# DataZooDE/anofox-forecast

Hardware: AMD Instinct MI355X
Metric: series/sec fit+forecast, AutoETS h=28 on M5-shape batches (higher is better)
Workload: dtype f64

## Files before the change

### anofox-forecast_amd/csrc/host_api.hip

```cpp
#include <hip/hip_runtime.h>

#include <algorithm>
#include <cctype>
#include <atomic>
#include <memory>
#include <unordered_map>
#include <chrono>
#include <cmath>
#include <condition_variable>
#include <mutex>
#include <cstdio>
#include <cstdlib>
#include <cstring>
#include <limits>
#include <map>
#include <stdexcept>
#include <string>
#include <system_error>
#include <thread>
#include <vector>

#include "classic_device.hpp"
#include "host_semantics.hpp"
#include "kernels.hpp"
// ... 59 lines not shown
    unsigned short *d_yc16 = nullptr;
    size_t yc_cells = 0;
    unsigned int *d_misfit = nullptr;
    unsigned int h_misfit[2] = {1u, 1u};
    int y_type = 0;
    unsigned long long *d_wave_trace = nullptr;
    unsigned long long *d_lane_stats = nullptr;
    double *d_yhat = nullptr, *d_lo = nullptr, *d_hi = nullptr;
    int32_t *d_model_code = nullptr, *d_status = nullptr, *d_detail = nullptr, *d_passes_total = nullptr, *d_evals_total = nullptr;
    uint32_t *d_mask = nullptr;
    int32_t *d_len_group = nullptr;
    int32_t *d_count = nullptr;
    int32_t *d_pos_map = nullptr, *d_pos_cnt = nullptr, *d_notpos = nullptr;
    double *d_ypos = nullptr;
    bool use_pos = false;
    bool none_pos = false;
    std::vector<anofox::FitArgs> insp_args;
    std::vector<anofox::FitLaunchers> insp_fns;
    std::vector<int> insp_spec, insp_stream;
    bool insp_ok = false;
    int insp_m = 1;
    int32_t live_pos = -1, live_all = -1;
    int arima_method = 0;
    size_t ar_ws_bytes = 0;
    double *ar_w = nullptr, *ar_wmean = nullptr, *ar_wsd = nullptr, *ar_l0 = nullptr, *ar_l1 = nullptr, *ar_x = nullptr, *ar_aicc = nullptr;
    int32_t *ar_wlen = nullptr, *ar_d = nullptr, *ar_D = nullptr, *ar_order = nullptr, *ar_status = nullptr, *ar_evals = nullptr, *ar_passes = nullptr, *ar_models = nullptr;
    StreamSet *sset = nullptr;
    hipStream_t own_stream = nullptr;
    hipStream_t aux[N_AUX_STREAMS] = {};
    hipEvent_t ev_start = nullptr, ev_stop = nullptr, ev_fit0 = nullptr, ev_fit1 = nullptr, ev_fork = nullptr;
    hipEvent_t ev_join[N_AUX_STREAMS] = {};
    struct Lane {
        double *ybuf = nullptr;
        size_t ybuf_cols = 0;
        int32_t *map[2] = {nullptr, nullptr};
        int32_t *cnt = nullptr;
        anofox::NmStateBuf st{};
        double *nm_scratch = nullptr;
        size_t nm_scratch_doubles = 0;
    } lanes[N_AUX_STREAMS];
    anofox::FitArgs *d_group_tab = nullptr, *h_group_tab = nullptr;
    size_t group_tab_cap = 0;
    hipEvent_t ev_group_tab = nullptr;
    hipStream_t last_stream = nullptr;
    bool ran = false, timed_fit = false;
    uint32_t fit_launches = 0;
    uint64_t n_problems = 0;
    Tunables tun;
    int seq_rounds = 3;
    int seq_rounds_env = -1;
    int spec_below_md = 8192;
    anofox::NmStateBuf classic_st{};
    int32_t *d_classic_status = nullptr, *classic_map[2] = {nullptr, nullptr}, *classic_cnt = nullptr;
    double *d_classic_ybuf = nullptr;
    size_t classic_ybuf_cols = 0;
    std::vector<void *> retired;
    int merged_m_max = 0;
    int32_t *d_m_col = nullptr;
    int spec2_below_md = 2048;
    int spec2_below = 1024;
    int spec_below = 8192;
    bool use_gather = false;
    double gather_budget = 0.0;
    bool sd_in_final = false;
    double *d_ring = nullptr;
    size_t ring_elems = 0;
    double *d_prep_scratch = nullptr;
    size_t prep_scratch_elems = 0;
    bool fixed_params = false;
    double fixed_x[4] = {0.0, 0.0, 0.0, 0.0};
    int32_t *d_im_level = nullptr, *d_im_gmax = nullptr;
    double *d_im_fc = nullptr;
    size_t im_fc_elems = 0;
// ... 124 lines not shown
{
    if (!b->sset) return;
    stream_set_give(b->sset);
    b->sset = nullptr; b->own_stream = nullptr; b->last_stream = nullptr; b->ran = false;
    for (auto &q : b->aux) q = nullptr;
}

void free_batch_buffers(AnofoxHipBatch *b)
{
    auto F = [](void *p) { dev_free(p, true); };
    if (b->owns_y) F(b->d_y);
    pin_free(b->h_stage);
    if (b->owns_len) F(b->d_len);
    F(b->d_mean); F(b->d_sd); F(b->d_fig_add); F(b->d_fig_mul); F(b->d_l0); F(b->d_b0); F(b->d_flags);
    F(b->d_aicc); F(b->d_yhat_slots); F(b->d_status_slots); F(b->d_evals_slots); F(b->d_iters_slots);
    F(b->d_passes_slots); F(b->d_slot_spec); F(b->d_lane_stats); F(b->d_wave_trace); F(b->d_yc32); F(b->d_yc16); F(b->d_misfit);
    F(b->d_yhat); F(b->d_lo); F(b->d_hi); F(b->d_model_code); F(b->d_status); F(b->d_detail);
    F(b->classic_st.sim); F(b->classic_st.fs); F(b->classic_st.phase); F(b->classic_st.evals); F(b->classic_st.iters); F(b->classic_st.passes); F(b->classic_st.done);
    F(b->d_classic_ybuf); F(b->d_classic_status); F(b->classic_map[0]); F(b->classic_map[1]); F(b->classic_cnt);
    for (void *p : b->retired) F(p);
    b->retired.clear();
    F(b->d_m_col); F(b->d_ring); F(b->d_prep_scratch);
    F(b->d_group_tab); pin_free(b->h_group_tab); b->d_group_tab = b->h_group_tab = nullptr; b->group_tab_cap = 0;
    if (b->ev_group_tab) { (void)hipEventDestroy(b->ev_group_tab); b->ev_group_tab = nullptr; }
    F(b->d_im_level); F(b->d_im_gmax); F(b->d_im_fc);
    F(b->d_th_sidx); F(b->d_th_adj);
    if (b->owns_exog) { F((void *)b->d_exog_x); F((void *)b->d_exog_f); }
    b->d_exog_x = b->d_exog_f = nullptr; b->owns_exog = false; b->exog_k = 0;
    F(b->d_exog_b0); F(b->d_exog_beta); F(b->d_exog_used);
    F(b->d_passes_total); F(b->d_evals_total); F(b->d_mask); F(b->d_len_group); F(b->d_count); F(b->d_pos_map); F(b->d_pos_cnt); F(b->d_notpos); F(b->d_ypos);
    F(b->ar_w); F(b->ar_wmean); F(b->ar_wsd); F(b->ar_l0); F(b->ar_l1); F(b->ar_x); F(b->ar_aicc); F(b->ar_wlen); F(b->ar_d); F(b->ar_D);
    F(b->ar_order); F(b->ar_status); F(b->ar_evals); F(b->ar_passes); F(b->ar_models);
    batch_detach_streams(b);
    for (auto &l : b->lanes) {
        F(l.ybuf); l.ybuf_cols = 0; F(l.map[0]); F(l.map[1]); F(l.cnt);
        F(l.st.sim); F(l.st.fs); F(l.st.phase); F(l.st.evals); F(l.st.iters); F(l.st.passes); F(l.st.done);
        F(l.nm_scratch); l.nm_scratch_doubles = 0;
    }
}

int max_slots_for(const Plan &p)
{
    if (p.model == M_AutoETS) return 30;
    if (p.model == M_ETS && p.ets_spec_id >= 0) return 1;
    return 0;
}

void alloc_common(AnofoxHipBatch *b)
{
    const size_t n = b->n, ld = b->ld, h = (size_t)std::max(b->h, 0);
    b->d_mean = dalloc<double>(ld);
    b->d_sd = dalloc<double>(ld);
    b->d_flags = dalloc<uint32_t>(ld);
    b->d_yhat = dalloc<double>(n * h);
    b->d_lo = dalloc<double>(n * h);
    b->d_hi = dalloc<double>(n * h);
    b->d_model_code = dalloc<int32_t>(ld);
    b->d_status = dalloc<int32_t>(ld);
    b->d_detail = dalloc<int32_t>(ld);
    b->d_passes_total = dalloc<int32_t>(ld);
    b->d_evals_total = dalloc<int32_t>(ld);
    b->d_mask = dalloc<uint32_t>(ld);
    b->d_len_group = dalloc<int32_t>(ld);
    b->d_count = dalloc<int32_t>(2);
    if (b->plan.model == M_AutoETS) {
        b->d_pos_map = dalloc<int32_t>(ld); b->d_pos_cnt = dalloc<int32_t>(2); b->d_notpos = dalloc<int32_t>(ld);
    }
    if (is_intermittent_model(b->plan.model)) {
// ... 2 lines not shown
    }
    if (is_theta_model(b->plan.model)) b->d_th_adj = dalloc<int32_t>(ld);
    if (b->plan.model == M_AutoARIMA) {
        const size_t T = std::max<size_t>(b->t_max, 1);
        b->ar_ws_bytes = arima_workspace_bytes((int)b->n, (int)T);
        b->ar_w = (double *)dalloc<char>(b->ar_ws_bytes);
        HIPCHECK(hipMemset(b->ar_w, 0, b->ar_ws_bytes));
        b->ar_wmean = dalloc<double>(ld); b->ar_wsd = dalloc<double>(ld); b->ar_l0 = dalloc<double>(ld); b->ar_l1 = dalloc<double>(ld);
        b->ar_x = dalloc<double>(6 * ld); b->ar_aicc = dalloc<double>(ld);
        b->ar_wlen = dalloc<int32_t>(ld); b->ar_d = dalloc<int32_t>(ld); b->ar_D = dalloc<int32_t>(ld); b->ar_order = dalloc<int32_t>(5 * ld);
        b->ar_status = dalloc<int32_t>(ld); b->ar_evals = dalloc<int32_t>(ld); b->ar_passes = dalloc<int32_t>(ld); b->ar_models = dalloc<int32_t>(ld);
        HIPCHECK(hipMemset(b->ar_wlen, 0, ld * sizeof(int32_t)));
    }
    HIPCHECK(hipMemset(b->d_model_code, 0, ld * sizeof(int32_t)));
    HIPCHECK(hipMemset(b->d_detail, 0, ld * sizeof(int32_t)));
    HIPCHECK(hipMemset(b->d_passes_total, 0, ld * sizeof(int32_t)));
    HIPCHECK(hipMemset(b->d_evals_total, 0, ld * sizeof(int32_t)));
    HIPCHECK(hipMemset(b->d_mask, 0, ld * sizeof(uint32_t)));
    b->n_slots_cap = max_slots_for(b->plan);
    if (b->n_slots_cap > 0) {
        const size_t S = (size_t)b->n_slots_cap;
        b->d_l0 = dalloc<double>(9 * ld);
        b->d_b0 = dalloc<double>(9 * ld);
        b->d_aicc = dalloc<double>(S * ld);
        b->d_yhat_slots = dalloc<double>(S * n * h);
        b->d_status_slots = dalloc<int32_t>(S * ld);
        b->d_evals_slots = dalloc<int32_t>(S * ld);
        b->d_iters_slots = dalloc<int32_t>(S * ld);
        b->d_passes_slots = dalloc<int32_t>(S * ld);
        b->d_slot_spec = dalloc<int32_t>(S);
        b->d_lane_stats = dalloc<unsigned long long>(2 * S);
        HIPCHECK(hipMemset(b->d_lane_stats, 0, 2 * S * sizeof(unsigned long long)));
        const int n_lanes = std::min<int>(N_AUX_STREAMS, b->n_slots_cap);
        for (int q = 0; q < n_lanes; q++) {
            auto &l = b->lanes[q];
            l.map[0] = dalloc<int32_t>(ld);
            l.map[1] = dalloc<int32_t>(ld);
            l.cnt = dalloc<int32_t>(3);
            l.st.sim = dalloc<double>(20 * ld);
            l.st.fs = dalloc<double>(5 * ld);
            l.st.phase = dalloc<int32_t>(ld);
            l.st.evals = dalloc<int32_t>(ld);
            l.st.iters = dalloc<int32_t>(ld);
            l.st.passes = dalloc<int32_t>(ld);
            l.st.done = dalloc<int32_t>(ld);
        }
    }
    batch_attach_streams(b);
}

void ensure_fig(AnofoxHipBatch *b, int m)
{
    if (m <= b->fig_m) return;
    if (b->d_fig_add) b->retired.push_back(b->d_fig_add);
    if (b->d_fig_mul) b->retired.push_back(b->d_fig_mul);
    b->d_fig_add = nullptr; b->d_fig_mul = nullptr; b->fig_m = 0;
    b->d_fig_add = dalloc<double>((size_t)m * b->ld);
    b->d_fig_mul = dalloc<double>((size_t)m * b->ld);
    b->fig_m = m;
}

double *ensure_ring(AnofoxHipBatch *b, size_t elems)
{
    if (b->ring_elems < elems) {
        if (b->d_ring) b->retired.push_back(b->d_ring);
        b->d_ring = nullptr; b->ring_elems = 0;
        b->d_ring = dalloc<double>(elems);
        b->ring_elems = elems;
    }
    return b->d_ring;
}
// ... 126 lines not shown
}

void batch_detect_periods(AnofoxHipBatch *b)
{
    std::vector<int32_t> per(b->n, 0);
    batch_attach_streams(b);
    detect_periods_block(b->d_y, b->ld, b->d_len, b->n, std::max<size_t>(b->t_max, 1), per.data(), b->own_stream);
    b->h_period.assign(b->n, 1);
    for (size_t s = 0; s < b->n; s++) b->h_period[s] = per[s] > 0 ? per[s] : 1;
}

void run_classic(AnofoxHipBatch *b, int kind, const int32_t *d_len, int m, int optimized, double alpha, int min_len,
                 const uint32_t *mask, uint32_t want, int32_t code, bool write_code, hipStream_t st)
{
    ClassicArgs a{};
    a.y = b->d_y; a.ld = b->ld; a.len = d_len; a.n_series = (int)b->n;
    a.m = m; a.h = b->h; a.optimized = optimized; a.fixed_alpha = alpha;
    a.mask = mask; a.want = want; a.min_len = min_len;
    a.yhat = b->d_yhat; a.status = b->d_detail; a.passes = b->d_passes_total;
    a.model_code = code; a.model_code_out = write_code ? b->d_model_code : nullptr;
    a.ring_scratch = nullptr;
    a.m_col = (kind == CK_HW || kind == CK_SEASONAL_ES) ? b->d_m_col : nullptr;
    const bool optimise = kind == CK_HOLT || kind == CK_HW || optimized != 0;
    if (optimise) {
        const size_t n = b->n, ld = b->ld;
        if (!b->classic_st.sim) {
            b->classic_st.sim = dalloc<double>(12 * ld); b->classic_st.fs = dalloc<double>(4 * ld);
            b->classic_st.phase = dalloc<int32_t>(ld); b->classic_st.evals = dalloc<int32_t>(ld); b->classic_st.iters = dalloc<int32_t>(ld);
            b->classic_st.passes = dalloc<int32_t>(ld); b->classic_st.done = dalloc<int32_t>(ld);
            b->d_classic_status = dalloc<int32_t>(ld);
            b->classic_map[0] = dalloc<int32_t>(ld); b->classic_map[1] = dalloc<int32_t>(ld); b->classic_cnt = dalloc<int32_t>(3);
        }
        double *ybuf = (b->n_slots_cap > 0 && b->use_gather) ? b->lanes[0].ybuf : nullptr;
        size_t ybuf_cols = ybuf ? b->lanes[0].ybuf_cols : ld;
        if (!ybuf) {
            const double per_col = (double)std::max<size_t>(b->t_max, 1) * 8.0;
            const size_t cols = (size_t)std::min((double)ld, 32.0 * 1073741824.0 / per_col) / 64 * 64;
            if (cols >= 1024 || cols >= ld) {
                if (!b->d_classic_ybuf) { b->d_classic_ybuf = dalloc<double>(std::max<size_t>(b->t_max, 1) * cols); b->classic_ybuf_cols = cols; }
                ybuf = b->d_classic_ybuf;
                ybuf_cols = b->classic_ybuf_cols;
            }
        }
        const bool seasonal = kind == CK_HW || kind == CK_SEASONAL_ES;
        FitArgs f{};
        f.y = b->d_y; f.ld = ld; f.len = d_len; f.n_series = (int)n; f.t_rows = (int)std::max<size_t>(b->t_max, 1);
        f.m = seasonal ? std::max(m, 1) : 1; f.h = b->h;
        f.flags = b->d_flags; f.fig = nullptr; f.fig_ld = ld;
        f.status = b->d_classic_status; f.st = b->classic_st;
        f.mask = mask; f.want = want; f.min_len = min_len;
        f.m_col = a.m_col;
        const bool merged = f.m_col != nullptr;
        FitLaunchers fns = classic_fit_launcher(kind, (merged && f.m == 7) ? 8 : f.m);
        if (!fns.round_seq || !fns.round_spec || !fns.round_spec2 || !fns.round_auto) throw HipFail{"no round kernel for this model"};
        if (f.m > ETS_LDS_PERIOD) {
            const size_t wg = merged ? n : std::max<size_t>((n + 15) / 16, std::min<size_t>(n, 1024));
            f.ring_scratch = ensure_ring(b, wg * (size_t)f.m * 64u);
            f.ring_scratch_doubles = wg * (size_t)f.m * 64u;
        }
        static const int BUDGET[] = {24, 24, 24, 24, 48, 48, 96, 192, 1024};
        const bool tiny = n <= TINY_BATCH_PROBLEMS;
        const int n_rounds = tiny ? 1 : (merged ? (n > 4096 ? 4 : 3) : (int)(sizeof BUDGET / sizeof BUDGET[0]));
        for (int r = 0; r < n_rounds; r++) {
            f.first_round = (r == 0);
            f.spec_below = -1; f.spec2_below = -1;
            f.gathered = 0;
            f.y_round = b->d_y; f.ld_round = ld; f.series_of = nullptr; f.n_active = nullptr;
// ... 291 lines not shown
                all_additive = false;
        int64_t additive_live = 0;
        for (size_t oi = 0; oi < order.size(); oi++)
            if (!dead[oi] && !spec_has_mult(specs[order[oi]])) additive_live += b->live_all >= 0 ? (int64_t)b->live_all : (int64_t)n;
        int64_t all_live = 0;
        for (size_t oi = 0; oi < order.size(); oi++)
            if (!dead[oi]) all_live += (spec_has_mult(specs[order[oi]]) && b->live_pos >= 0) ? (int64_t)b->live_pos : (b->live_all >= 0 ? (int64_t)b->live_all : (int64_t)n);
        const bool on = b->tun.k4 > 0 || (b->tun.k4 < 0 && yt == YT_F64 && ((all_additive && additive_live >= 131072) || all_live >= 524288));
        for (size_t oi = 0; oi < order.size(); oi++)
            k4[oi] = on && !dead[oi] && !b->fixed_params && !spec_has_mult(specs[order[oi]]) && fns[oi].round_k4 && fns[oi].round_auto_k4;
    }
    std::vector<char> fill_spec4(order.size(), 0);
    bool fill_mode = false;
    {
        int64_t lanes = 0;
        std::vector<int64_t> live_of(order.size(), 0);
        for (size_t oi = 0; oi < order.size(); oi++) {
            if (dead[oi]) continue;
            live_of[oi] = (spec_has_mult(specs[order[oi]]) && b->live_pos >= 0) ? (int64_t)b->live_pos : (b->live_all >= 0 ? (int64_t)b->live_all : (int64_t)n);
            lanes += live_of[oi];
        }
        const int64_t resident = 2 * 1024 * 64;
        const bool tiny_batch = (uint64_t)n * order.size() <= (uint64_t)TINY_BATCH_PROBLEMS;
        fill_mode = b->tun.fill_policy > 0 && !tiny_batch && !b->fixed_params && order.size() > 1 && b->seq_rounds_env < 0 && b->seq_rounds == 0 &&
                    lanes * 4 > 8 * resident;
        if (fill_mode) {
            const int64_t target = resident * (int64_t)b->tun.fill_target / 100;
            for (size_t oi = 0; oi < order.size(); oi++) {
                if (dead[oi] || k4[oi]) continue;
                if (lanes + 3 * live_of[oi] <= target) { fill_spec4[oi] = 1; lanes += 3 * live_of[oi]; }
            }
        }
    }
    if (b->use_gather && !b->fixed_params) {
        const size_t T = std::max<size_t>(b->t_max, 1);
        std::vector<size_t> need(order.size(), 0);
        double total = 0.0;
        for (size_t oi = 0; oi < order.size(); oi++) {
            if (dead[oi]) continue;
            size_t c = (b->use_pos && args[oi].need_positive && b->live_pos >= 0) ? (size_t)b->live_pos : n;
            need[oi] = std::min(ld, (c + 63) / 64 * 64);
            total += (double)need[oi] * (double)T * 8.0;
        }
        const double scale = total > b->gather_budget ? b->gather_budget / total : 1.0;
        for (size_t oi = 0; oi < order.size(); oi++) {
            if (dead[oi]) continue;
            auto &lane = b->lanes[oi % (size_t)n_lanes];
            size_t cols = scale < 1.0 ? (size_t)((double)need[oi] * scale) / 64 * 64 : need[oi];
            if (b->tun.gather_cols > 0) cols = std::min<size_t>(need[oi], (size_t)b->tun.gather_cols / 64 * 64);
            if (cols < need[oi] && cols < 1024 && b->tun.gather_cols <= 0) cols = 0;
            if (lane.ybuf && lane.ybuf_cols >= cols) continue;
            if (lane.ybuf) {
                HIPCHECK(hipDeviceSynchronize());
                dev_free(lane.ybuf, true);
                lane.ybuf = nullptr; lane.ybuf_cols = 0;
            }
            while (cols >= 64) {
                try { lane.ybuf = dalloc<double>(T * cols); lane.ybuf_cols = cols; break; }
                catch (const HipFail &f) {
                    if (!f.oom) throw;
                    cols = cols / 2 / 64 * 64;
                    if (cols < 1024) cols = 0;
                }
            }
        }
    }
    const bool tiny = (uint64_t)n * order.size() <= (uint64_t)TINY_BATCH_PROBLEMS;
    const int total_rounds = b->fixed_params ? 0 : (tiny ? 1 : n_rounds);
    enum { RK_SEQ, RK_SPEC, RK_SPEC2, RK_AUTO, RK_K4, RK_AUTO_K4 };
    std::vector<int> group_of(order.size(), -1);
    std::vector<std::vector<size_t>> groups;
    std::vector<int> group_stream;
    std::vector<GroupLaunchFn> group_fn;
    std::vector<size_t> slot_of(order.size(), 0);
    size_t n_slots = 0;
    bool grouped = b->tun.group_launch > 0 && !inline_stream && !tiny && !merged && !b->fixed_params && total_rounds > 0;
    if (grouped) {
        GroupLaunchFn fn[N_GROUP_CLASSES];
        for (int c = 0; c < N_GROUP_CLASSES; c++) fn[c] = ets_group_launcher(c, m, yt);
        std::vector<size_t> of_class[N_GROUP_CLASSES];
        for (size_t oi = 0; oi < order.size() && grouped; oi++) {
            if (dead[oi]) continue;
            const int c = ets_group_class(specs[order[oi]]);
            if (c < 0 || !fn[c] || fns[oi].nm_scratch_per_wg != 0) grouped = false;
            else of_class[c].push_back(oi);
        }
        if (grouped) {
            auto add = [&](const std::vector<size_t> &sl, int c) {
                if (sl.empty()) return;
                if (sl.size() > (size_t)GROUP_MAX_SLOTS) throw HipFail{"launch_fit_slots: more specs in one group than GROUP_MAX_SLOTS"};
                groups.push_back(sl); group_fn.push_back(fn[c]);
// ... 60 lines not shown
            const bool spec_mode = r >= b->seq_rounds;
            a.first_round = (r == 0);
            a.wave_trace_tag = ((unsigned long long)specs[order[oi]] << 32) | ((unsigned long long)r << 16);
            a.wave_prio = (int)oi < b->tun.prio_top ? std::max(1, 3 - (int)oi) : 0;
            a.spec_below = -1; a.spec2_below = -1;
            a.gathered = 0;
            if (tiny) {
                a.y_round = b->d_y; a.ld_round = ld; a.series_of = nullptr; a.n_active = nullptr;
                a.budget = 1 << 30; a.budget_seq = a.budget;
                run_round(oi, RK_SPEC2, a, sq, r);
                b->fit_launches++;
                return;
            }
            if (r == 0 && b->use_pos && a.need_positive) {
                if (emit)
                    hipLaunchKernelGGL(retire_nonpositive_kernel, dim3((unsigned)((n + 255) / 256)), dim3(256), 0, sq, (int)n, d_len, b->d_notpos,
                                       a.status, lane.st.done, lane.st.passes, lane.st.evals, lane.st.iters);
                a.series_of = b->d_pos_map; a.n_active = b->d_pos_cnt;
                if (b->d_ypos) { a.y_round = b->d_ypos; a.ld_round = ld; a.gathered = 1; a.gather_cap = (int)ld; }
                else { a.y_round = b->d_y; a.ld_round = ld; }
            } else if (r == 0) {
                a.y_round = a.y; a.ld_round = ld; a.series_of = nullptr; a.n_active = nullptr;
            } else {
                const int32_t *prev_map = (r == 1) ? nullptr : lane.map[(r - 1) & 1];
                const int32_t *prev_cnt = (r == 1) ? nullptr : lane.cnt + ((r - 1) % 3);
                if (emit && !grouped && r == 1) HIPCHECK(hipMemsetAsync(lane.cnt, 0, 3 * sizeof(int32_t), sq));
                if (emit && !grouped) launch_compact(prev_map, prev_cnt, (int)n, lane.st.done, lane.map[r & 1], lane.cnt + (r % 3), sq, lane.cnt + ((r + 1) % 3));
                if (emit && grouped) {
                    const int k = gc.n_slots++;
                    gc.prev[k] = prev_map; gc.n_prev[k] = prev_cnt; gc.done[k] = lane.st.done;
                    gc.next[k] = lane.map[r & 1]; gc.n_next[k] = lane.cnt + (r % 3); gc.n_clear[k] = lane.cnt + ((r + 1) % 3);
                }
                a.series_of = lane.map[r & 1]; a.n_active = lane.cnt + (r % 3);
                if (b->use_gather && lane.ybuf) {
                    if (emit && !grouped)
                        launch_gather_columns(a.y, ld, lane.map[r & 1], lane.cnt + (r % 3), (int)n, (int)b->t_max, lane.ybuf, lane.ybuf_cols, sq,
                                              (int)lane.ybuf_cols, ybytes);
                    if (emit && grouped) {
                        const int k = gg.n_slots++;
                        gg.series_of[k] = lane.map[r & 1]; gg.n_active[k] = lane.cnt + (r % 3);
                        gg.out[k] = lane.ybuf; gg.ld_out[k] = lane.ybuf_cols; gg.cap[k] = (int)lane.ybuf_cols;
                        gg_cols = std::max(gg_cols, (int)std::min<size_t>(n, lane.ybuf_cols));
                    }
                    a.y_round = lane.ybuf; a.ld_round = lane.ybuf_cols; a.gathered = 1; a.gather_cap = (int)lane.ybuf_cols;
                } else {
                    a.y_round = a.y; a.ld_round = ld;
                }
            }
            const int s2 = (spec_trend_idx(specs[order[oi]]) == 4) ? b->spec2_below_md : b->spec2_below;
            if (fill_mode && !k4[oi]) {
                const int64_t live_i = (spec_has_mult(specs[order[oi]]) && b->live_pos >= 0) ? (int64_t)b->live_pos : (b->live_all >= 0 ? (int64_t)b->live_all : (int64_t)n);
                const int s2v = (int)std::max<int64_t>(32, std::min<int64_t>(s2 > 0 ? s2 : 32, live_i / std::max(1, b->tun.fill_s2_div)));
                a.budget = BUDGET[r]; a.budget_seq = (BUDGET[r] * 7) / 4;
                if (r == 0) {
                    if (fill_spec4[oi]) run_round(oi, RK_SPEC, a, sq, r);
                    else { a.budget = a.budget_seq; run_round(oi, RK_SEQ, a, sq, r); }
                } else {
                    a.spec_below = fill_spec4[oi] ? 0x7fffffff : (int)std::max<int64_t>(64, live_i / std::max(1, b->tun.fill_late_div));
                    a.spec2_below = s2v;
                    run_round(oi, RK_AUTO, a, sq, r);
                }
                if (!grouped) b->fit_launches++;
                return;
            }
            if (k4[oi]) {
                a.budget = BUDGET[r]; a.budget_seq = BUDGET[r];
                const int64_t live = b->live_all >= 0 ? b->live_all : (int64_t)n;
                const int sb = ((int)oi < b->tun.k4_top && b->tun.k4_top_below > 0) ? b->tun.k4_top_below : b->spec_below;
                if (r == 0) run_round(oi, live > sb ? RK_K4 : RK_SPEC, a, sq, r);
                else {
                    a.spec_below = sb; a.spec2_below = s2 > 0 ? s2 : -1;
                    run_round(oi, RK_AUTO_K4, a, sq, r);
                }
            } else if (r == 0 || b->seq_rounds_env >= 0 || b->seq_rounds == 0) {
                a.budget = spec_mode ? BUDGET[r] : (BUDGET[r] * 7) / 4;
                if (spec_mode && r > 0 && s2 > 0) {
                    a.spec_below = 0x7fffffff; a.spec2_below = s2; a.budget_seq = a.budget;
                    run_round(oi, RK_AUTO, a, sq, r);
                } else
                    run_round(oi, spec_mode ? RK_SPEC : RK_SEQ, a, sq, r);
            } else {
                a.spec_below = (spec_trend_idx(specs[order[oi]]) == 4) ? b->spec_below_md : b->spec_below;
                a.spec2_below = s2 > 0 ? s2 : -1;
                if ((int)oi < b->tun.top_boost_n) {
                    a.spec_below = (int)std::min<int64_t>(0x7fffffff, (int64_t)a.spec_below * b->tun.top_boost_pct / 100);
                    if (a.spec2_below > 0) a.spec2_below = (int)std::min<int64_t>(0x7fffffff, (int64_t)a.spec2_below * b->tun.top_boost_pct / 100);
                }
                a.budget_seq = (BUDGET[r] * 7) / 4;
                a.budget = BUDGET[r];
                run_round(oi, RK_AUTO, a, sq, r);
            }
            if (!grouped) b->fit_launches++;
    };
    if (grouped) {
        const size_t cells = (size_t)total_rounds * n_slots;
        if (b->ev_group_tab) HIPCHECK(hipEventSynchronize(b->ev_group_tab));
        else HIPCHECK(hipEventCreateWithFlags(&b->ev_group_tab, hipEventDisableTiming));
        if (b->group_tab_cap < cells) {
            if (b->d_group_tab) b->retired.push_back(b->d_group_tab);
            pin_free(b->h_group_tab);
            b->d_group_tab = nullptr; b->h_group_tab = nullptr; b->group_tab_cap = 0;
            b->d_group_tab = dalloc<FitArgs>(cells);
            b->h_group_tab = (FitArgs *)pin_alloc_bytes(cells * sizeof(FitArgs));
            b->group_tab_cap = cells;
        }
        slot_blocks.assign(cells, 0); slot_k4.assign(cells, 0);
        emit = false;
        for (int r = 0; r < total_rounds; r++) for (size_t oi = 0; oi < order.size(); oi++) enqueue_round(r, oi);
        emit = true;
        HIPCHECK(hipMemcpyAsync(b->d_group_tab, b->h_group_tab, cells * sizeof(FitArgs), hipMemcpyHostToDevice, st));
        HIPCHECK(hipEventRecord(b->ev_group_tab, st));
        HIPCHECK(hipEventRecord(b->ev_fork, st));
        for (int q : group_stream) HIPCHECK(hipStreamWaitEvent(b->aux[q], b->ev_fork, 0));
    } else
        for (int i = 0; i < n_fork; i++) HIPCHECK(hipStreamWaitEvent(b->aux[i], b->ev_fit0, 0));
    for (size_t oi = 0; oi < order.size(); oi++)
        if (dead[oi]) {
            const FitArgs &a = args[oi];
            hipLaunchKernelGGL(retire_nonpositive_kernel, dim3((unsigned)((n + 255) / 256)), dim3(256), 0, spec_stream(stream_of[oi]), (int)n, d_len,
                               b->d_notpos, a.status, a.st.done, a.st.passes, a.st.evals, a.st.iters, a.aicc, a.passes, a.evals, a.iters);
        }
    if (b->fixed_params) {
        for (size_t oi = 0; oi < order.size(); oi++) {
            const int id = specs[order[oi]];
            FitArgs &a = args[oi];
            double x[4] = {0.0, 0.0, 0.0, 0.0};
            int d = 0;
            x[d++] = b->fixed_x[0];
            if (spec_trend_idx(id) != 0) x[d++] = b->fixed_x[1];
            if (spec_season(id) != 0) x[d++] = b->fixed_x[2];
            if (spec_trend_idx(id) == 2 || spec_trend_idx(id) == 4) x[d++] = b->fixed_x[3];
            hipLaunchKernelGGL(ets_fixed_setup_kernel, dim3((unsigned)((n + 255) / 256)), dim3(256), 0, spec_stream(stream_of[oi]), (int)n, ld, d_len,
                               b->d_flags, spec_season(id) != 0 ? 1 : 0, a.m, a.n_param, a.need_positive, d, x[0], x[1], x[2], x[3], a.status,
                               a.st.sim, a.st.evals, a.st.iters, a.st.passes, a.st.done);
        }
        LAUNCHCHECK("ETS fixed-parameter setup");
    }
    auto enqueue_group_round = [&](const int r, const size_t g) {
        hipStream_t sg = b->aux[group_stream[g]];
        if (r == 0) {
            int32_t *zero[GROUP_MAX_SLOTS] = {};
            for (size_t k = 0; k < groups[g].size(); k++) zero[k] = b->lanes[groups[g][k] % (size_t)n_lanes].cnt;
            launch_group_zero3((int)groups[g].size(), zero, sg);
        }
        gc = GroupCompactArgs{}; gc.n_series = (int)n;
        gg = GroupGatherArgs{}; gg.t_max = (int)b->t_max; gg.elem_bytes = ybytes; gg.y = ybase; gg.ld = ld; gg_cols = 0;
        for (size_t oi : groups[g]) enqueue_round(r, oi);
        if (gc.n_slots > 0) launch_group_compact(gc, sg);
        if (gg.n_slots > 0) launch_group_gather(gg, gg_cols, sg);
        GroupRoundArgs ga{};
        ga.n_slots = (int)groups[g].size();
        const size_t row = (size_t)r * n_slots + slot_of[groups[g][0]];
        for (int k = 0; k < ga.n_slots; k++) {
            const size_t oi = groups[g][(size_t)k];
            ga.spec[k] = specs[order[oi]];
            ga.k4[k] = slot_k4[(size_t)r * n_slots + slot_of[oi]];
            ga.start[k + 1] = ga.start[k] + slot_blocks[(size_t)r * n_slots + slot_of[oi]];
        }
        group_fn[g](b->d_group_tab + row, ga, m, sg);
        b->fit_launches++;
    };
    int head = 0;
    if (grouped && total_rounds > 0 && b->tun.dm_head_rounds > 0 && groups.size() > 1 && group_stream[0] == 0 &&
        spec_trend_idx(specs[order[groups[0][0]]]) == 4) {
        head = std::min(b->tun.dm_head_rounds, total_rounds);
        for (int r = 0; r < head; r++) enqueue_group_round(r, 0);
        LAUNCHCHECK("ETS fit head rounds");
        HIPCHECK(hipEventRecord(b->ev_join[0], b->aux[0]));
        for (size_t g = 1; g < groups.size(); g++) HIPCHECK(hipStreamWaitEvent(b->aux[group_stream[g]], b->ev_join[0], 0));
    } else if (!grouped && !tiny && !inline_stream && total_rounds > 0 && b->tun.dm_head_rounds > 0) {
        std::vector<size_t> dm, rest;
        for (size_t oi = 0; oi < order.size(); oi++)
            if (!dead[oi]) (spec_trend_idx(specs[order[oi]]) == 4 ? dm : rest).push_back(oi);
        if (!dm.empty() && !rest.empty()) {
            head = std::min(b->tun.dm_head_rounds, total_rounds);
            for (int r = 0; r < head; r++) for (size_t oi : dm) enqueue_round(r, oi);
            LAUNCHCHECK("ETS fit head rounds");
// ... 4810 lines not shown
```

### anofox-forecast_amd/csrc/host_resources.hpp

```cpp
#pragma once

constexpr int N_AUX_STREAMS = 32;

struct HipFail { std::string msg; bool oom = false; };
void report_hip_failure(AnofoxError *out_error, const HipFail &f)
{
    if (f.oom) anofox::set_error(out_error, ALLOCATION_ERROR, "Allocation error: " + f.msg);
    else anofox::set_error(out_error, INTERNAL_ERROR, "Internal error: " + f.msg);
}
#define HIPCHECK(expr)                                                                             \
    do {                                                                                           \
        hipError_t _e = (expr);                                                                    \
        if (_e != hipSuccess) throw HipFail{std::string(#expr) + ": " + hipGetErrorString(_e), _e == hipErrorOutOfMemory};    \
    } while (0)

#define LAUNCHCHECK(what)                                                                          \
    do {                                                                                           \
        hipError_t _e = hipGetLastError();                                                         \
        if (_e != hipSuccess) throw HipFail{std::string("kernel launch failed (") + (what) + "): " + hipGetErrorString(_e), false};    \
    } while (0)

constexpr int32_t STATUS_NOT_COMPUTED = -1;

struct Tunables {
    std::vector<int> budgets{24, 24, 24, 24, 24, 24, 48, 48, 96, 96, 192, 1024};
    int seq_rounds = -1;
    int gather_cols = 0;
    int gather = -1;
    int spec_below = 8192;
    int spec_below_md = 8192;
    int spec2_below = 1024;
    int spec2_below_md = 2048;
    int k4 = -1;
    int k4_top = 1, k4_top_below = 20480;
    std::string wave_trace;
    int compact = -1;
    int fill_policy = 1;
    int fill_target = 150;
    int fill_late_div = 2;
    int fill_s2_div = 16;
    int top_boost_n = 0, top_boost_pct = 200;
    int prio_top = 0;
    int group_launch = 1;
    int group_split = 1;
    int dm_head_rounds = 0;
    bool merge_periods = true;
    int part_threads = 16;
    int pack_threads = 0;
    bool timing = false;
    int arima_trace = 0;
    double arima_lookahead = 6.0;
    int arima_lookahead_depth = 2;
    double arima_spec_factor = 4.0;
    double arima_shared_chunk_rounds = 1.0;
    int arima_prep_lanes = 64;
    int arima_queue_sort = 1;
    int arima_refit_budget = 100;
    static std::map<std::string, std::string> tune_map()
    {
        std::map<std::string, std::string> kv;
        const char *e = std::getenv("ANOFOX_HIP_TUNE");
// ... 8 lines not shown
                std::string k = item.substr(0, eq), v = item.substr(eq + 1);
                while (!k.empty() && k.front() == ' ') k.erase(k.begin());
                while (!k.empty() && k.back() == ' ') k.pop_back();
                kv[k] = v;
            }
            pos = end + 1;
        }
        return kv;
    }
    static Tunables from_env()
    {
        Tunables t;
        const std::map<std::string, std::string> kv = tune_map();
        auto geti = [&](const char *k, int &v) { auto it = kv.find(k); if (it != kv.end()) v = std::atoi(it->second.c_str()); };
        auto getd = [&](const char *k, double &v) { auto it = kv.find(k); if (it != kv.end()) v = std::atof(it->second.c_str()); };
        if (kv.count("budgets")) {
            std::vector<int> v;
            for (const char *q = kv.at("budgets").c_str(); *q;) {
                char *end = nullptr;
                long x = std::strtol(q, &end, 10);
                if (end == q) break;
                if (x > 0) v.push_back((int)x);
                q = (*end == ',') ? end + 1 : end;
            }
            if (!v.empty()) t.budgets = v;
        }
        if (kv.count("wave_trace")) t.wave_trace = kv.at("wave_trace");
        geti("compact", t.compact); geti("prio_top", t.prio_top); geti("top_boost_n", t.top_boost_n); geti("top_boost_pct", t.top_boost_pct);
        geti("fill_policy", t.fill_policy); geti("fill_target", t.fill_target); geti("fill_late_div", t.fill_late_div); geti("fill_s2_div", t.fill_s2_div);
        geti("seq_rounds", t.seq_rounds);
        geti("gather", t.gather);
        if (kv.count("spec_below")) t.spec_below = t.spec_below_md = std::atoi(kv.at("spec_below").c_str());
        geti("spec_below_md", t.spec_below_md);
        geti("gather_cols", t.gather_cols);
        geti("group_launch", t.group_launch); geti("group_split", t.group_split);
        geti("k4", t.k4); geti("dm_head_rounds", t.dm_head_rounds); geti("k4_top", t.k4_top); geti("k4_top_below", t.k4_top_below);
        if (kv.count("spec2_below")) t.spec2_below = t.spec2_below_md = std::atoi(kv.at("spec2_below").c_str());
        geti("spec2_below_md", t.spec2_below_md);
        if (kv.count("merge_periods")) t.merge_periods = std::atoi(kv.at("merge_periods").c_str()) != 0;
        geti("part_threads", t.part_threads);
        if (kv.count("arima_trace")) t.arima_trace = std::atoi(kv.at("arima_trace").c_str());
        getd("arima_lookahead", t.arima_lookahead);
        geti("arima_lookahead_depth", t.arima_lookahead_depth);
        getd("arima_spec_factor", t.arima_spec_factor);
        geti("arima_queue_sort", t.arima_queue_sort);
        geti("arima_prep_lanes", t.arima_prep_lanes);
        getd("arima_shared_chunk_rounds", t.arima_shared_chunk_rounds);
        geti("arima_refit_budget", t.arima_refit_budget);
        if (const char *e = std::getenv("ANOFOX_HIP_PACK_THREADS")) t.pack_threads = std::max(1, std::atoi(e));
        t.timing = std::getenv("ANOFOX_HIP_TIMING") != nullptr;
        return t;
    }
};
struct ProcessTunables {
    double cache_gb = -1.0, pinned_cache_gb = 2.0;
    double coalesce_us = 1000.0;
    int prio_streams = -1;
    std::string devices;
    static const ProcessTunables &get()
    {
        static const ProcessTunables t = [] {
            ProcessTunables p;
            if (const char *e = std::getenv("ANOFOX_HIP_CACHE_GB")) p.cache_gb = std::atof(e);
            if (const char *e = std::getenv("ANOFOX_HIP_PINNED_CACHE_GB")) p.pinned_cache_gb = std::atof(e);
            { const auto kv = Tunables::tune_map(); auto it = kv.find("prio_streams"); if (it != kv.end()) p.prio_streams = std::atoi(it->second.c_str()); }
            if (const char *e = std::getenv("ANOFOX_HIP_COALESCE_US")) p.coalesce_us = std::atof(e);
            if (const char *e = std::getenv("ANOFOX_HIP_DEVICES")) p.devices = e;
// ... 427 lines not shown
```

### anofox-forecast_amd/csrc/kernels.hip

```cpp
#include "classic_device.hpp"
#include "fit_units.hpp"
#include "kernels.hpp"

namespace anofox {

__global__ __launch_bounds__(NM_BLOCK) void select_kernel(const SelectArgs a)
{
    const int s = blockIdx.x * NM_BLOCK + threadIdx.x;
    if (s >= a.n_series) return;
    if (a.len[s] <= 0) { a.fallback_mask[s] = 0u; return; }
    int best = -1;
    double best_aicc = __builtin_huge_val();
    int passes = 0, evals = 0;
    for (int k = 0; k < a.n_slots; k++) {
        passes += a.passes_slots[(size_t)k * a.ld + s];
        evals += a.evals_slots[(size_t)k * a.ld + s];
        if (a.status_slots[(size_t)k * a.ld + s] != FIT_OK) continue;
        double v = a.aicc[(size_t)k * a.ld + s];
        if (v < best_aicc) { best_aicc = v; best = k; }
    }
    a.passes_total[s] = passes;
    a.evals_total[s] = evals;
    if (best < 0) {
        a.status[s] = -1;
// ... 270 lines not shown

constexpr int GROUP_COMPACT_BLOCKS = 256, GROUP_GATHER_COL_BLOCKS = 128, GROUP_GATHER_ROW_BLOCKS = 8;
__global__ __launch_bounds__(NM_BLOCK) void group_compact_kernel(const GroupCompactArgs g)
{
    const int k = blockIdx.y;
    if (g.n_clear[k] && blockIdx.x == 0 && threadIdx.x == 0) *g.n_clear[k] = 0;
    const int n_prev = g.n_prev[k] ? *g.n_prev[k] : g.n_series;
    const int32_t *prev = g.prev[k], *done = g.done[k];
    const int lane = threadIdx.x;
    for (int base0 = (int)blockIdx.x * NM_BLOCK; base0 < n_prev; base0 += (int)gridDim.x * NM_BLOCK) {
        const int idx = base0 + lane;
        int s = 0;
        bool keep = false;
        if (idx < n_prev) {
            s = prev ? prev[idx] : idx;
            keep = done[s] == 0;
        }
        const unsigned long long bal = __ballot(keep);
        const int cnt = __popcll(bal);
        if (cnt == 0) continue;
        int base = 0;
        if (lane == 0) base = atomicAdd(g.n_next[k], cnt);
        base = __shfl(base, 0);
        const int before = __popcll(bal & ((1ull << lane) - 1ull));
        if (keep) g.next[k][base + before] = s;
    }
}

void launch_group_compact(const GroupCompactArgs &g, hipStream_t stream)
{
    if (g.n_slots <= 0 || g.n_series <= 0) return;
    const int grid = std::min((g.n_series + NM_BLOCK - 1) / NM_BLOCK, GROUP_COMPACT_BLOCKS);
    hipLaunchKernelGGL(group_compact_kernel, dim3(grid, g.n_slots), dim3(NM_BLOCK), 0, stream, g);
}

struct GroupZeroArgs { int32_t *p[GROUP_MAX_SLOTS]; };
__global__ void group_zero3_kernel(const int n, const GroupZeroArgs z)
{
    const int i = threadIdx.x;
    if (i < 3 * n) z.p[i / 3][i % 3] = 0;
}

void launch_group_zero3(int n, int32_t *const *zero, hipStream_t stream)
{
    if (n <= 0) return;
    GroupZeroArgs z{};
    for (int k = 0; k < n && k < GROUP_MAX_SLOTS; k++) z.p[k] = zero[k];
    hipLaunchKernelGGL(group_zero3_kernel, dim3(1), dim3(64), 0, stream, std::min(n, GROUP_MAX_SLOTS), z);
}

template <class E>
__global__ __launch_bounds__(NM_BLOCK) void group_gather_kernel(const GroupGatherArgs g)
{
    const int k = blockIdx.z;
    const int n_act = *g.n_active[k];
    if (n_act > g.cap[k]) return;
    const E *y = (const E *)g.y;
    E *out = (E *)g.out[k];
    const size_t ld_out = g.ld_out[k];
    const int32_t *series_of = g.series_of[k];
    for (int p0 = (int)blockIdx.x * NM_BLOCK; p0 < n_act; p0 += (int)gridDim.x * NM_BLOCK) {
        const int p = p0 + (int)threadIdx.x;
        const int s = series_of[p < n_act ? p : n_act - 1];
        for (int t0 = (int)blockIdx.y * GATHER_TB; t0 < g.t_max; t0 += (int)gridDim.y * GATHER_TB) {
            const int t1 = t0 + GATHER_TB < g.t_max ? t0 + GATHER_TB : g.t_max;
            for (int t = t0; t < t1; t++) out[(size_t)t * ld_out + p] = y[(size_t)t * g.ld + s];
        }
    }
}

void launch_group_gather(const GroupGatherArgs &g, int n_cols_max, hipStream_t stream)
{
    if (g.n_slots <= 0 || g.t_max <= 0 || n_cols_max <= 0) return;
    dim3 grid(std::min((n_cols_max + NM_BLOCK - 1) / NM_BLOCK, GROUP_GATHER_COL_BLOCKS),
              std::min((g.t_max + GATHER_TB - 1) / GATHER_TB, GROUP_GATHER_ROW_BLOCKS), g.n_slots);
    if (g.elem_bytes == 8) hipLaunchKernelGGL(group_gather_kernel<double>, grid, dim3(NM_BLOCK), 0, stream, g);
    else if (g.elem_bytes == 4) hipLaunchKernelGGL(group_gather_kernel<float>, grid, dim3(NM_BLOCK), 0, stream, g);
    else hipLaunchKernelGGL(group_gather_kernel<unsigned short>, grid, dim3(NM_BLOCK), 0, stream, g);
}

__global__ __launch_bounds__(NM_BLOCK) void compact_block_kernel(const double *y, size_t ld, const int32_t *len, int n_series, int t_rows, float *out32,
// ... 154 lines not shown
```

### anofox-forecast_amd/csrc/kernels.hpp

```cpp
#pragma once
#include <hip/hip_runtime.h>
#include <stddef.h>
#include <stdint.h>
#include <atomic>

#include <stdexcept>
#include <string>

namespace anofox {

inline void anofox_check_attr(hipError_t e)
{
    if (e != hipSuccess) throw std::runtime_error(std::string("launch preparation failed: ") + hipGetErrorString(e));
}

enum : uint32_t { SF_POSITIVE = 1u, SF_CONSTANT = 2u, SF_HAS_NAN = 4u };

enum : int32_t { FIT_OK = 0, FIT_SHORT = 1, FIT_NONPOSITIVE = 2, FIT_NONFINITE = 3, FIT_PERIOD = 4, FIT_SKIPPED = 5 };

struct PrepArgs {
    const double *y; size_t ld; const int32_t *len; int n_series;
    int m;
    const int32_t *m_col;
    double *mean, *sd;
// ... 392 lines not shown
};

typedef void (*FitLaunchFn)(const FitArgs &, hipStream_t);
struct FitLaunchers { FitLaunchFn round_seq, round_spec, round_spec2, round_auto, final; size_t nm_scratch_per_wg; FitLaunchFn round_k4, round_auto_k4; };
constexpr int ETS_PERLANE_LDS = -3, ETS_PERLANE_HBM = -4;
FitLaunchers ets_fit_launcher(int spec_id, int m, int yt = 0);
constexpr int GROUP_MAX_SLOTS = 16;
enum { GROUP_DAMPED_MUL = 0, GROUP_GENERAL = 1, GROUP_ADDITIVE = 2, N_GROUP_CLASSES = 3 };
struct GroupRoundArgs {
    int n_slots;
    int spec[GROUP_MAX_SLOTS];
    int k4[GROUP_MAX_SLOTS];
    int start[GROUP_MAX_SLOTS + 1];
};
typedef void (*GroupLaunchFn)(const FitArgs *tab, const GroupRoundArgs &g, int m, hipStream_t);
GroupLaunchFn ets_group_launcher(int group_class, int m, int yt);
inline int ets_group_class(int spec_id)
{
    if (spec_id < 0 || spec_id >= 30 || (spec_id >= 15 && spec_id % 3 == 1)) return -1;
    const int e = spec_id / 15, ti = (spec_id % 15) / 3, s = spec_id % 3;
    if (ti == 4) return GROUP_DAMPED_MUL;
    return (e == 0 && ti < 3 && s < 2) ? GROUP_ADDITIVE : GROUP_GENERAL;
}
FitLaunchers classic_fit_launcher(int kind, int m);
struct ClassicArgs;
void launch_classic_final(int kind, const FitArgs &a, const ClassicArgs &c, hipStream_t stream);

struct GroupCompactArgs {
    int n_slots, n_series;
    const int32_t *prev[GROUP_MAX_SLOTS], *n_prev[GROUP_MAX_SLOTS], *done[GROUP_MAX_SLOTS];
    int32_t *next[GROUP_MAX_SLOTS], *n_next[GROUP_MAX_SLOTS], *n_clear[GROUP_MAX_SLOTS];
};
void launch_group_compact(const GroupCompactArgs &g, hipStream_t);
void launch_group_zero3(int n, int32_t *const *zero, hipStream_t);
struct GroupGatherArgs {
    int n_slots, t_max, elem_bytes;
    const void *y; size_t ld;
    const int32_t *series_of[GROUP_MAX_SLOTS], *n_active[GROUP_MAX_SLOTS];
    void *out[GROUP_MAX_SLOTS]; size_t ld_out[GROUP_MAX_SLOTS]; int cap[GROUP_MAX_SLOTS];
};
void launch_group_gather(const GroupGatherArgs &g, int n_cols_max, hipStream_t);
void launch_compact(const int32_t *series_prev, const int32_t *n_prev, int n_series, const int32_t *done,
                    int32_t *series_next, int32_t *n_next, hipStream_t, int32_t *n_clear = nullptr);
constexpr int DETECT_LDS_ROWS = 8192;
constexpr int DETECT_LONG_GRID = 1024;
size_t detect_scratch_doubles(int n_series, int t_rows);
void launch_detect_periods(const double *y, size_t ld, const int32_t *len, int n_series, int t_rows, double *scratch, int32_t *period,
                           double *best_acf, hipStream_t stream);
void launch_gather_columns(const void *y, size_t ld, const int32_t *series_of, const int32_t *n_active, int n_series,
                           int t_max, void *out, size_t ld_out, hipStream_t stream, int cap, int elem_bytes = 8);
void launch_compact_block(const double *y, size_t ld, const int32_t *len, int n_series, int t_rows, float *out32, unsigned short *out16,
                          unsigned int *misfit, hipStream_t stream);

struct ArimaArgs {
    const double *y; size_t ld; const int32_t *len; int n_series;
    int m, h;
    int t_max;
    void *ws; size_t ws_bytes;
    int32_t *wlen, *d, *D;
    double *wmean, *wsd, *last_d0, *last_d1;
    int32_t *order;
    double *xbest;
    double *aicc;
    int32_t *status, *evals, *passes, *models;
    double *yhat;
    int32_t *model_code;
    int trace;
// ... 26 lines not shown
```

Before: 81840.

## Pack lane counters, zero with one memset, resize gather buffers by bytes

Lane counter triples now live in one contiguous device allocation. A single async memset before the fork clears them, replacing the per-group zero3 kernel launch on each aux stream. Gather buffers are tracked by bytes and sized by element width, so a buffer is reused whenever it is large enough instead of being reallocated. A per-spec gather column cap is added, with an optional gather_below_pct knob (default 100, inactive) to limit gathered columns. This cuts kernel launches and reallocation syncs, at the cost of more complex capacity bookkeeping.

```diff
diff --git a/anofox-forecast_amd/csrc/host_api.hip b/anofox-forecast_amd/csrc/host_api.hip
--- a/anofox-forecast_amd/csrc/host_api.hip
+++ b/anofox-forecast_amd/csrc/host_api.hip
@@ -115,6 +115,7 @@
     hipEvent_t ev_join[N_AUX_STREAMS] = {};
     struct Lane {
         double *ybuf = nullptr;
+        size_t ybuf_bytes = 0;
         size_t ybuf_cols = 0;
         int32_t *map[2] = {nullptr, nullptr};
         int32_t *cnt = nullptr;
@@ -122,6 +123,7 @@
         double *nm_scratch = nullptr;
         size_t nm_scratch_doubles = 0;
     } lanes[N_AUX_STREAMS];
+    int32_t *d_lane_cnt = nullptr;
     anofox::FitArgs *d_group_tab = nullptr, *h_group_tab = nullptr;
     size_t group_tab_cap = 0;
     hipEvent_t ev_group_tab = nullptr;
@@ -312,8 +314,9 @@
     F(b->ar_w); F(b->ar_wmean); F(b->ar_wsd); F(b->ar_l0); F(b->ar_l1); F(b->ar_x); F(b->ar_aicc); F(b->ar_wlen); F(b->ar_d); F(b->ar_D);
     F(b->ar_order); F(b->ar_status); F(b->ar_evals); F(b->ar_passes); F(b->ar_models);
     batch_detach_streams(b);
+    F(b->d_lane_cnt); b->d_lane_cnt = nullptr;
     for (auto &l : b->lanes) {
-        F(l.ybuf); l.ybuf_cols = 0; F(l.map[0]); F(l.map[1]); F(l.cnt);
+        F(l.ybuf); l.ybuf_cols = 0; l.ybuf_bytes = 0; F(l.map[0]); F(l.map[1]); l.cnt = nullptr;
         F(l.st.sim); F(l.st.fs); F(l.st.phase); F(l.st.evals); F(l.st.iters); F(l.st.passes); F(l.st.done);
         F(l.nm_scratch); l.nm_scratch_doubles = 0;
     }
@@ -382,11 +385,12 @@
         b->d_lane_stats = dalloc<unsigned long long>(2 * S);
         HIPCHECK(hipMemset(b->d_lane_stats, 0, 2 * S * sizeof(unsigned long long)));
         const int n_lanes = std::min<int>(N_AUX_STREAMS, b->n_slots_cap);
+        b->d_lane_cnt = dalloc<int32_t>(3 * (size_t)n_lanes);
         for (int q = 0; q < n_lanes; q++) {
             auto &l = b->lanes[q];
             l.map[0] = dalloc<int32_t>(ld);
             l.map[1] = dalloc<int32_t>(ld);
-            l.cnt = dalloc<int32_t>(3);
+            l.cnt = b->d_lane_cnt + 3 * q;
             l.st.sim = dalloc<double>(20 * ld);
             l.st.fs = dalloc<double>(5 * ld);
             l.st.phase = dalloc<int32_t>(ld);
@@ -579,7 +583,8 @@
             b->classic_map[0] = dalloc<int32_t>(ld); b->classic_map[1] = dalloc<int32_t>(ld); b->classic_cnt = dalloc<int32_t>(3);
         }
         double *ybuf = (b->n_slots_cap > 0 && b->use_gather) ? b->lanes[0].ybuf : nullptr;
-        size_t ybuf_cols = ybuf ? b->lanes[0].ybuf_cols : ld;
+        size_t ybuf_cols = ybuf ? std::min(ld, b->lanes[0].ybuf_bytes / (std::max<size_t>(b->t_max, 1) * sizeof(double)) / 64 * 64) : ld;
+        if (ybuf && ybuf_cols < 64) { ybuf = nullptr; ybuf_cols = ld; }
         if (!ybuf) {
             const double per_col = (double)std::max<size_t>(b->t_max, 1) * 8.0;
             const size_t cols = (size_t)std::min((double)ld, 32.0 * 1073741824.0 / per_col) / 64 * 64;
@@ -937,15 +942,21 @@
             }
         }
     }
+    std::vector<int> gather_cap(order.size(), 0);
     if (b->use_gather && !b->fixed_params) {
         const size_t T = std::max<size_t>(b->t_max, 1);
+        const int pct = std::min(100, std::max(0, b->tun.gather_below_pct));
         std::vector<size_t> need(order.size(), 0);
         double total = 0.0;
         for (size_t oi = 0; oi < order.size(); oi++) {
             if (dead[oi]) continue;
             size_t c = (b->use_pos && args[oi].need_positive && b->live_pos >= 0) ? (size_t)b->live_pos : n;
             need[oi] = std::min(ld, (c + 63) / 64 * 64);
-            total += (double)need[oi] * (double)T * 8.0;
+            if (pct < 100) {
+                const size_t start = (args[oi].need_positive && b->live_pos >= 0) ? (size_t)b->live_pos : (b->live_all >= 0 ? (size_t)b->live_all : n);
+                need[oi] = std::min(need[oi], start * (size_t)pct / 100 / 64 * 64);
+            }
+            total += (double)need[oi] * (double)T * (double)ybytes;
         }
         const double scale = total > b->gather_budget ? b->gather_budget / total : 1.0;
         for (size_t oi = 0; oi < order.size(); oi++) {
@@ -954,14 +965,22 @@
             size_t cols = scale < 1.0 ? (size_t)((double)need[oi] * scale) / 64 * 64 : need[oi];
             if (b->tun.gather_cols > 0) cols = std::min<size_t>(need[oi], (size_t)b->tun.gather_cols / 64 * 64);
             if (cols < need[oi] && cols < 1024 && b->tun.gather_cols <= 0) cols = 0;
-            if (lane.ybuf && lane.ybuf_cols >= cols) continue;
+            if (cols < 64) continue;
+            if (lane.ybuf && lane.ybuf_bytes >= T * cols * (size_t)ybytes) {
+                lane.ybuf_cols = cols; gather_cap[oi] = (int)cols;
+                continue;
+            }
             if (lane.ybuf) {
                 HIPCHECK(hipDeviceSynchronize());
                 dev_free(lane.ybuf, true);
-                lane.ybuf = nullptr; lane.ybuf_cols = 0;
+                lane.ybuf = nullptr; lane.ybuf_cols = 0; lane.ybuf_bytes = 0;
             }
             while (cols >= 64) {
-                try { lane.ybuf = dalloc<double>(T * cols); lane.ybuf_cols = cols; break; }
+                try {
+                    lane.ybuf = (double *)dalloc<char>(T * cols * (size_t)ybytes);
+                    lane.ybuf_bytes = T * cols * (size_t)ybytes; lane.ybuf_cols = cols; gather_cap[oi] = (int)cols;
+                    break;
+                }
                 catch (const HipFail &f) {
                     if (!f.oom) throw;
                     cols = cols / 2 / 64 * 64;
@@ -1088,17 +1107,17 @@
                     gc.next[k] = lane.map[r & 1]; gc.n_next[k] = lane.cnt + (r % 3); gc.n_clear[k] = lane.cnt + ((r + 1) % 3);
                 }
                 a.series_of = lane.map[r & 1]; a.n_active = lane.cnt + (r % 3);
-                if (b->use_gather && lane.ybuf) {
+                if (b->use_gather && lane.ybuf && gather_cap[oi] > 0) {
+                    const int cap = gather_cap[oi];
                     if (emit && !grouped)
-                        launch_gather_columns(a.y, ld, lane.map[r & 1], lane.cnt + (r % 3), (int)n, (int)b->t_max, lane.ybuf, lane.ybuf_cols, sq,
-                                              (int)lane.ybuf_cols, ybytes);
+                        launch_gather_columns(a.y, ld, lane.map[r & 1], lane.cnt + (r % 3), (int)n, (int)b->t_max, lane.ybuf, (size_t)cap, sq, cap, ybytes);
                     if (emit && grouped) {
                         const int k = gg.n_slots++;
                         gg.series_of[k] = lane.map[r & 1]; gg.n_active[k] = lane.cnt + (r % 3);
-                        gg.out[k] = lane.ybuf; gg.ld_out[k] = lane.ybuf_cols; gg.cap[k] = (int)lane.ybuf_cols;
-                        gg_cols = std::max(gg_cols, (int)std::min<size_t>(n, lane.ybuf_cols));
+                        gg.out[k] = lane.ybuf; gg.ld_out[k] = (size_t)cap; gg.cap[k] = cap;
+                        gg_cols = std::max(gg_cols, std::min((int)n, cap));
                     }
-                    a.y_round = lane.ybuf; a.ld_round = lane.ybuf_cols; a.gathered = 1; a.gather_cap = (int)lane.ybuf_cols;
+                    a.y_round = lane.ybuf; a.ld_round = (size_t)cap; a.gathered = 1; a.gather_cap = cap;
                 } else {
                     a.y_round = a.y; a.ld_round = ld;
                 }
@@ -1165,6 +1184,7 @@
         for (int r = 0; r < total_rounds; r++) for (size_t oi = 0; oi < order.size(); oi++) enqueue_round(r, oi);
         emit = true;
         HIPCHECK(hipMemcpyAsync(b->d_group_tab, b->h_group_tab, cells * sizeof(FitArgs), hipMemcpyHostToDevice, st));
+        HIPCHECK(hipMemsetAsync(b->d_lane_cnt, 0, 3 * (size_t)n_lanes * sizeof(int32_t), st));
         HIPCHECK(hipEventRecord(b->ev_group_tab, st));
         HIPCHECK(hipEventRecord(b->ev_fork, st));
         for (int q : group_stream) HIPCHECK(hipStreamWaitEvent(b->aux[q], b->ev_fork, 0));
@@ -1194,11 +1214,6 @@
     }
     auto enqueue_group_round = [&](const int r, const size_t g) {
         hipStream_t sg = b->aux[group_stream[g]];
-        if (r == 0) {
-            int32_t *zero[GROUP_MAX_SLOTS] = {};
-            for (size_t k = 0; k < groups[g].size(); k++) zero[k] = b->lanes[groups[g][k] % (size_t)n_lanes].cnt;
-            launch_group_zero3((int)groups[g].size(), zero, sg);
-        }
         gc = GroupCompactArgs{}; gc.n_series = (int)n;
         gg = GroupGatherArgs{}; gg.t_max = (int)b->t_max; gg.elem_bytes = ybytes; gg.y = ybase; gg.ld = ld; gg_cols = 0;
         for (size_t oi : groups[g]) enqueue_round(r, oi);
diff --git a/anofox-forecast_amd/csrc/host_resources.hpp b/anofox-forecast_amd/csrc/host_resources.hpp
--- a/anofox-forecast_amd/csrc/host_resources.hpp
+++ b/anofox-forecast_amd/csrc/host_resources.hpp
@@ -27,6 +27,7 @@
     int seq_rounds = -1;
     int gather_cols = 0;
     int gather = -1;
+    int gather_below_pct = 100;
     int spec_below = 8192;
     int spec_below_md = 8192;
     int spec2_below = 1024;
@@ -101,7 +102,7 @@
         geti("gather", t.gather);
         if (kv.count("spec_below")) t.spec_below = t.spec_below_md = std::atoi(kv.at("spec_below").c_str());
         geti("spec_below_md", t.spec_below_md);
-        geti("gather_cols", t.gather_cols);
+        geti("gather_cols", t.gather_cols); geti("gather_below_pct", t.gather_below_pct);
         geti("group_launch", t.group_launch); geti("group_split", t.group_split);
         geti("k4", t.k4); geti("dm_head_rounds", t.dm_head_rounds); geti("k4_top", t.k4_top); geti("k4_top_below", t.k4_top_below);
         if (kv.count("spec2_below")) t.spec2_below = t.spec2_below_md = std::atoi(kv.at("spec2_below").c_str());
diff --git a/anofox-forecast_amd/csrc/kernels.hip b/anofox-forecast_amd/csrc/kernels.hip
--- a/anofox-forecast_amd/csrc/kernels.hip
+++ b/anofox-forecast_amd/csrc/kernels.hip
@@ -326,21 +326,6 @@
     if (g.n_slots <= 0 || g.n_series <= 0) return;
     const int grid = std::min((g.n_series + NM_BLOCK - 1) / NM_BLOCK, GROUP_COMPACT_BLOCKS);
     hipLaunchKernelGGL(group_compact_kernel, dim3(grid, g.n_slots), dim3(NM_BLOCK), 0, stream, g);
-}
-
-struct GroupZeroArgs { int32_t *p[GROUP_MAX_SLOTS]; };
-__global__ void group_zero3_kernel(const int n, const GroupZeroArgs z)
-{
-    const int i = threadIdx.x;
-    if (i < 3 * n) z.p[i / 3][i % 3] = 0;
-}
-
-void launch_group_zero3(int n, int32_t *const *zero, hipStream_t stream)
-{
-    if (n <= 0) return;
-    GroupZeroArgs z{};
-    for (int k = 0; k < n && k < GROUP_MAX_SLOTS; k++) z.p[k] = zero[k];
-    hipLaunchKernelGGL(group_zero3_kernel, dim3(1), dim3(64), 0, stream, std::min(n, GROUP_MAX_SLOTS), z);
 }
 
 template <class E>
diff --git a/anofox-forecast_amd/csrc/kernels.hpp b/anofox-forecast_amd/csrc/kernels.hpp
--- a/anofox-forecast_amd/csrc/kernels.hpp
+++ b/anofox-forecast_amd/csrc/kernels.hpp
@@ -448,7 +448,6 @@
     int32_t *next[GROUP_MAX_SLOTS], *n_next[GROUP_MAX_SLOTS], *n_clear[GROUP_MAX_SLOTS];
 };
 void launch_group_compact(const GroupCompactArgs &g, hipStream_t);
-void launch_group_zero3(int n, int32_t *const *zero, hipStream_t);
 struct GroupGatherArgs {
     int n_slots, t_max, elem_bytes;
     const void *y; size_t ld;
```

Result: slower. 80910 (-1.1%).
